# yangt1013/SPEINet

Hardware: AMD Instinct MI355X
Metric: deblurred 720p frames/sec (higher is better)
Workload: dtype f16 (correlation top2)

## Files before the change

### include/speinet_hip.h

```cpp
#ifndef SPEINET_HIP_H
#define SPEINET_HIP_H

#include <stdint.h>

#ifdef __cplusplus
extern "C" {
#endif

typedef void* spei_stream_t;

#define SPEI_ACT_NONE 0
#define SPEI_ACT_RELU 1
#define SPEI_ACT_GELU 2

#define SPEI_F32 0
#define SPEI_BF16 1
#define SPEI_F16 2

#define SPEI_CONV 0
#define SPEI_CONV_TRANSPOSED 1

int spei_version(void);
const char* spei_last_error(void);
const char* spei_arch(void);

int spei_any_nonzero(const float* x, int64_t n, int32_t* flag, spei_stream_t stream);

int spei_rl_prior(const float* img, float* out, float* scratch, int C, int H, int W, int iters, float lam,
                  spei_stream_t stream);

int spei_conv5_in(const float* img_chw, const float* w, const float* bias, float* out_hwc, int H, int W,
                  int Cout, spei_stream_t stream);

int spei_conv5_out(const float* in_hwc, int ldi, const float* w, const float* bias, float* out_chw, int H,
                   int W, int Cin, spei_stream_t stream);

int spei_igemm_f32(const float* a0, int lda0, int k0, const float* a1, int lda1, int k1, const float* w,
                   const float* bias, float* out, int ldo, const float* residual, int ldr,
                   const float* rowscale, int Hin, int Win, int Hout, int Wout, int N, int ksize, int stride,
                   int pad, int mode, int act, spei_stream_t stream);

int spei_igemm_f32_batched(const float* a0, int lda0, int k0, const float* a1, int lda1, int k1, const float* w,
                           const float* bias, float* out, int ldo, const float* residual, int ldr,
                           const float* rowscale, int Hin, int Win, int Hout, int Wout, int N, int ksize, int stride,
                           int pad, int mode, int act, int batch, spei_stream_t stream);

int spei_conv_slab16(int fmt, const void* a0, int lda0, int k0, const void* a1, int lda1, int k1, int a_fmt,
                     const void* wfrag_hi, const void* wfrag_lo, const float* bias, void* out, int ldo, int out_fmt,
                     const float* residual, int ldr, const float* rowscale, int Hin, int Win, int Hout, int Wout,
                     int N, int ksize, int stride, int pad, int act, int ln_input, spei_stream_t stream);

int spei_conv_slab16_batched(int fmt, const void* a0, int k0, int a_fmt, const void* wfrag, const void* wfrag_lo, const float* bias,
                             void* out, int out_fmt, const float* residual, int batch, int Hin, int Win, int Hout, int Wout, int N,
                             int ksize, int stride, int pad, int act, spei_stream_t stream);

int spei_conv32_ws16(int fmt, const void* a, int a_fmt, const void* wfrag, const float* bias, void* out, int out_fmt, int batch,
                     int H, int W, int act, spei_stream_t stream);

int spei_conv64_ws16(int fmt, const void* a, int a_fmt, const void* wfrag, const float* bias, void* out, int out_fmt, int batch,
                     int H, int W, int act, spei_stream_t stream);

int spei_mlp_fused16(int fmt, const float* x, float* out, const void* w1_frag, const float* b1, const void* w2_frag,
                     const float* b2, int64_t M, spei_stream_t stream);

int spei_convt2_slab16(int fmt, const void* a0, int lda0, int k0, int a_fmt, const void* wfrag00, const void* wfrag01,
                       const void* wfrag10, const void* wfrag11, const float* bias, void* out, int ldo, int out_fmt,
                       int Hin, int Win, int N, int act, spei_stream_t stream);

int spei_convt2_slab16x3(const float* a0, int lda0, int k0, const void* const* whi4, const void* const* wlo4, const float* bias,
                         float* out, int ldo, int Hin, int Win, int N, int act, spei_stream_t stream);

int spei_conv3x3_256_pipe16(int fmt, const float* x, const void* w_frag, const float* bias, const float* residual, float* out,
                            int batch, int H, int W, spei_stream_t stream);

int spei_conv5_out_slab16(int fmt, const void* in, int ldi, int in_fmt, const void* wfrag, const float* bias32, float* out_chw,
                          int H, int W, spei_stream_t stream);

int spei_attn_fused16(int fmt, const float* x, float* out, const void* yhat, const void* wq_frag, const float* bq,
                      const void* wkv_frag, const float* bkv, const void* wproj_frag, const float* bproj,
                      const float* relbias, int H, int W, int shift, spei_stream_t stream);

int spei_attn_win4_16(int fmt, const float* x, float* out, const void* yhat, const void* wq_frag, const float* bq,
                      const void* wkv_frag, const float* bkv, const void* wproj_frag, const float* bproj,
                      const float* relbias, int batch, int H, int W, int shift, spei_stream_t stream);

int64_t spei_frame_metrics_ws_doubles(int H, int W, int border);
int spei_frame_metrics(const unsigned char* out_hwc, const unsigned char* gt_hwc, int H, int W, int border, double* ws, double* result,
                       spei_stream_t stream);

int64_t spei_gate_ws_floats(int H, int W, int C);
int spei_resblock_gates(const void* x1, int x1_fmt, int H, int W, int C, const float* se_w1, const float* se_b1,
                        const float* se_w2, const float* se_b2, const float* cw_w, const float* cw_bn,
                        const float* hc_w, const float* hc_bn, float* s, float* g1, float* g2, float* ws,
                        spei_stream_t stream);
int spei_resblock_apply(const float* x, const void* x1, int x1_fmt, const float* s, const float* g1, const float* g2,
                        const float* extra, float* out, int ldo, int H, int W, int C, spei_stream_t stream);

int spei_resblock_gates_batched(const void* x1, int x1_fmt, int batch, int H, int W, int C, const float* se_w1, const float* se_b1,
                                const float* se_w2, const float* se_b2, const float* cw_w, const float* cw_bn, const float* hc_w,
                                const float* hc_bn, float* s, float* g1, float* g2, float* ws, spei_stream_t stream);
int spei_resblock_apply_batched(const float* x, const void* x1, int x1_fmt, const float* s, const float* g1, const float* g2, float* out,
                                int batch, int H, int W, int C, spei_stream_t stream);

int spei_layernorm256(const float* x, void* y, int out_fmt, const float* gamma, const float* beta, int64_t M,
                      spei_stream_t stream);

int spei_window_attention(const void* q, const void* kv, int io_fmt, const float* relbias, void* out, int H, int W,
                          int shift, spei_stream_t stream);
int spei_window_attention_batched(const void* q, const void* kv, int io_fmt, const float* relbias, void* out, int H, int W,
                                  int shift, int batch, spei_stream_t stream);

int spei_patch_invnorm(const float* f, int ldf, float* inv, int H, int W, int C, spei_stream_t stream);

int64_t spei_corr_ws_floats(int64_t n_lr);
int spei_corr_argmax(const float* lr, int ldl, const float* ref, int ldr, const float* inv_lr,
                     const float* inv_ref, int Hl, int Wl, int Hr, int Wr, int C, float* S, int32_t* arg,
                     float* ws, spei_stream_t stream);

int spei_split16(int fmt, const float* x, int ld, void* hi, void* lo, int64_t M, int C, spei_stream_t stream);
int spei_corr_argmax_bf16(const void* lr_hi, const void* lr_lo, const void* ref_hi, const void* ref_lo,
                          const float* inv_lr, const float* inv_ref, int Hl, int Wl, int Hr, int Wr, int C, float* S,
                          int32_t* arg, float* ws, spei_stream_t stream);

int spei_corr_slab16(int fmt, const void* lr_hi, const void* lr_lo, const void* ref_hi, const void* ref_lo,
                     const float* inv_lr, const float* inv_ref, int Hl, int Wl, int Hr, int Wr, int C, float* S,
                     int32_t* arg, float* ws, spei_stream_t stream);

int spei_corr_slab_top2_16(int fmt, const void* lr16, const void* ref16, const float* inv_lr, const float* inv_ref,
                           int Hl, int Wl, int Hr, int Wr, int C, float* S, int32_t* arg, float* S2, int32_t* arg2,
                           float* ws, spei_stream_t stream);
int64_t spei_corr_diag_ws_floats(int Hl, int Wl, int Hr, int Wr);
int spei_corr_diag_top2_16(int fmt, const void* lr16, const void* ref16, const float* inv_ref, int Hl, int Wl, int Hr, int Wr,
                           int C, float* S, int32_t* arg, float* S2, int32_t* arg2, float* ws, spei_stream_t stream);
int spei_corr_rescore(const float* lr, int ldl, const float* ref, int ldr, const float* inv_lr, const float* inv_ref,
                      int Hl, int Wl, int Hr, int Wr, int C, float* S, int32_t* arg, const float* S2, const int32_t* arg2,
                      spei_stream_t stream);

int spei_gather_fold(const float* ref, int ldr, const int32_t* arg, float* out, int ldo, int H3, int W3,
                     int Hr3, int Wr3, int C, int s, spei_stream_t stream);

int spei_rot90(const float* in, int ldi, float* out, int H, int W, int C, spei_stream_t stream);

int spei_upsample_bicubic(const float* in, int ldi, float* out, int ldo, int H, int W, int C, int s, int act,
// ... 119 lines not shown
```

### speinet_amd/engine.py

```python
from __future__ import annotations

import torch

from .ops import ACT_GELU, ACT_RELU, CONV_T, BMap, Ctx, FMap


def _resblocks(ctx: Ctx, f: FMap, blocks, extra=None, out=None) -> FMap:
    n = len(blocks)
    for i, pk in enumerate(blocks):
        last = i == n - 1
        f = ctx.resblock(f, pk, extra=extra if last else None, out=out if last else None)
    return f


def in_block(ctx: Ctx, frame: torch.Tensor, pk: dict) -> FMap:
    ctx = ctx.for_stage("enc")
    return _resblocks(ctx, ctx.conv5_in(frame, pk["head_w"], pk["head_b"]), pk["blocks"])


def enc_stage(ctx: Ctx, f: FMap, pk: dict, extra=None, out=None) -> FMap:
    ctx = ctx.for_stage("enc")
    n = pk["head_b"].numel()
    f = ctx.igemm(f, pk["head_w"], pk["head_b"], n, ksize=5, stride=2, act=ACT_RELU)
    return _resblocks(ctx, f, pk["blocks"], extra, out)
# ... 86 lines not shown
        ctx.igemm(FMap(cur, h, w, 256), layer["conv_w"], layer["conv_b"], 256, ksize=3, residual=rf, out=rf)
    xt = ctx.layernorm(r, sw["norm_g"], sw["norm_b"])
    res = ctx.igemm(FMap(xt, h, w, 256), sw["cab_w"], sw["cab_b"], 256, ksize=3, residual=sx.x_first)
    return ctx.igemm(res, sw["conv_last_w"], sw["conv_last_b"], 128, ksize=3, residual=sx.f_mid, out=out)


def swin_multi(ctx: Ctx, sx: SwinX, feats: BMap, sw: dict, outs: list) -> None:
    ctx = ctx.for_stage("swin")
    B, h, w = feats.B, feats.H, feats.W
    m = h * w
    dev = feats.t.device
    y_first = ctx.igemm_batched(feats, sw["conv_first_w"], sw["conv_first_b"], 256, 3)
    yt = ctx.layernorm(y_first.t, sw["pe_g"], sw["pe_b"])
    idt = ctx.inter_dtype()
    yhat = ctx.layernorm(yt, out_dtype=idt)
    del y_first, yt
    r = sx.xt0.repeat(B, 1)
    bufs = [torch.empty(B * m, 256, device=dev), torch.empty(B * m, 256, device=dev)]
    for layer in sw["layers"]:
        cur = r
        for bi, bk in enumerate(layer["blocks"]):
            shift = 0 if bi % 2 == 0 else 2
            nxt = bufs[bi % 2]
            ctx.attn_fused(cur, yhat, bk, h, w, shift, out=nxt)
            ctx.mlp_fused(nxt, bk["w1"], bk["b1"], bk["w2"], bk["b2"], out=nxt)
            cur = nxt
        rb = BMap(r, B, h, w, 256)
        ctx.igemm_batched(BMap(cur, B, h, w, 256), layer["conv_w"], layer["conv_b"], 256, 3, residual=rb, out=rb)
    xt = ctx.layernorm(r, sw["norm_g"], sw["norm_b"])
    x_first = BMap(sx.x_first.t.repeat(B, 1), B, h, w, 256)
    res = ctx.igemm_batched(BMap(xt, B, h, w, 256), sw["cab_w"], sw["cab_b"], 256, 3, residual=x_first)
    for b in range(B):
        ctx.igemm(res.map(b), sw["conv_last_w"], sw["conv_last_b"], 128, ksize=3, residual=sx.f_mid, out=outs[b])


def search_plan(ctx: Ctx, f_fusion: FMap, lv3: FMap):
    ctx = ctx.for_stage("search")
    return ctx.corr_plan(f_fusion, lv3, ctx.patch_invnorm(f_fusion), ctx.patch_invnorm(lv3))


def search_finish(ctx: Ctx, plan, f_fusion: FMap, lv1: FMap, lv2: FMap, lv3: FMap, return_arg=False):
    ctx = ctx.for_stage("search")
    s, arg = plan.s, plan.arg
    if ctx.capture is not None:
        ctx.capture.update(arg=arg, s=s)
    h3, w3 = f_fusion.H, f_fusion.W
    t3 = ctx.gather_fold(lv3, arg, h3, w3, lv3.H, lv3.W, 1)
    t2 = ctx.gather_fold(lv2, arg, h3, w3, lv3.H, lv3.W, 2)
    t1 = ctx.gather_fold(lv1, arg, h3, w3, lv3.H, lv3.W, 4)
    if return_arg:
        return s, t3, t2, t1, arg
    return s, t3, t2, t1


def search_transfer(ctx: Ctx, f_fusion: FMap, lv1: FMap, lv2: FMap, lv3: FMap, return_arg=False):
    plan = search_plan(ctx, f_fusion, lv3)
    plan.launch()
    return search_finish(ctx, plan, f_fusion, lv1, lv2, lv3, return_arg)


def self_plan(ctx: Ctx, f_fusion: FMap):
    ctx = ctx.for_stage("search")
    ref = ctx.rot90(f_fusion)
    return ctx.corr_plan(f_fusion, ref, ctx.patch_invnorm(f_fusion), ctx.patch_invnorm(ref))


def self_finish(ctx: Ctx, plan, f_fusion: FMap, P: dict):
    ctx = ctx.for_stage("search")
    s = plan.s
    if ctx.capture is not None:
        ctx.capture.update(s_self=s)
    p1, p2 = P["SelfTransfer.search1"], P["SelfTransfer.search2"]
    t2 = ctx.up_conv1x1_relu(f_fusion, p1["w"], p1["b"], 64)
    t1 = ctx.up_conv1x1_relu(t2, p2["w"], p2["b"], 32)
    return s, f_fusion, t2, t1


def self_transfer(ctx: Ctx, f_fusion: FMap, P: dict):
    plan = self_plan(ctx, f_fusion)
    plan.launch()
    return self_finish(ctx, plan, f_fusion, P)


def decode(ctx: Ctx, ff: FMap, s: torch.Tensor, t3: FMap, t2: FMap, t1: FMap, P: dict, out: torch.Tensor) -> torch.Tensor:
    ctx = ctx.for_stage("decode")
    g = ctx.for_stage("glue")
    g1 = ctx.for_stage("glue1")
    c = lambda name: (P[name]["w"], P[name]["b"])
    h3, w3 = ff.H, ff.W
    smap = FMap(s.view(h3 * w3, 1), h3, w3, 1)
    f_lv3 = g.igemm(ff, *c("conv_lv3"), 128, a1=t3, rowscale=s, residual=ff)
    dec2 = dec_stage(ctx.for_stage("dec2"), f_lv3, P["decoder_second"])
    s2 = ctx.upsample(smap, 2).t.view(-1)
    f_lv2 = g.igemm(dec2, *c("conv_lv2"), 64, a1=t2, rowscale=s2, residual=dec2)
    s1 = g.up_conv1x1_relu(f_lv3, *c("search1"), 64)
    sr2 = g.igemm(f_lv2, *c("search3"), 64, ksize=3, act=ACT_RELU)
    f_v3 = g.igemm(dec2, *c("search2"), 64, a1=s1, act=ACT_RELU, residual=dec2)
    f_lv2 = g.igemm(f_lv2, *c("search2"), 64, a1=sr2, act=ACT_RELU, residual=f_lv2)
    dec1 = dec_stage(ctx.for_stage("dec1"), f_lv2, P["decoder_first"])
    s4 = ctx.upsample(smap, 4).t.view(-1)
    f_lv1 = g1.igemm(dec1, *c("conv_lv1"), 32, a1=t1, rowscale=s4, residual=dec1)
    s13 = g.up_conv1x1_relu(f_v3, *c("search13"), 32)
    s23 = g1.igemm(ctx.upsample(f_lv2, 2), *c("search33"), 32, ksize=3, act=ACT_RELU)
    s33 = g1.igemm(f_lv1, *c("search43"), 32, ksize=3, act=ACT_RELU)
    acc = g1.igemm(s13, *c("search33"), 32, ksize=3, a1=s23, act=ACT_RELU, residual=f_lv1)
    g1.igemm(s13, *c("search33"), 32, ksize=3, a1=s33, act=ACT_RELU, residual=acc, out=acc)
    g1.igemm(s23, *c("search33"), 32, ksize=3, a1=s33, act=ACT_RELU, residual=acc, out=acc)
    ob = P["outBlock"]
    ctx = ctx.for_stage("out")
    f = _resblocks(ctx, acc, ob["blocks"])
    return ctx.for_stage("tail").conv5_out(f, ob["tail_w"], ob["tail_b"], out, ob.get("tail_w32"), ob.get("tail_b32"))


def _lanes(ctx: Ctx, sides) -> list:
    return [torch.cuda.current_stream(ctx.device)] + list(sides or ())


def forward_sample(ctx: Ctx, x: torch.Tensor, P: dict, n_seq: int, has_ref: bool, out: torch.Tensor, sides=()) -> torch.Tensor:
    return _run(forward_sample_steps(ctx, x, P, n_seq, has_ref, out, sides), out)


def _run(steps, out):
    for plan in steps:
        plan.launch()
    return out


def forward_sample_steps(ctx: Ctx, x: torch.Tensor, P: dict, n_seq: int, has_ref: bool, out: torch.Tensor, sides=()):
    h, w = x.shape[-2:]
    h3, w3 = h // 4, w // 4
    dev = x.device
    lanes = _lanes(ctx, sides)
    main = lanes[0]
    if ctx.for_stage("enc").batched_available():
        yield from forward_batch_steps(ctx, x[None], P, n_seq, [not has_ref], out[None], sides)
        return
    for s_ in lanes[1:]:
        s_.wait_stream(main)
    lv = None
    if has_ref:
        with torch.cuda.stream(lanes[-1]):
            lv = reference_pyramid(ctx, x[n_seq + 1], P)
    cat = FMap(torch.empty(h3 * w3, 128 * n_seq, device=dev), h3, w3, 128 * n_seq)
    mid = x[n_seq // 2]
    e0 = enc(ctx, mid, P)
    f_mid = enc(ctx, ctx.rl_prior(mid, 5, 0.01), P, extra=e0, out=cat.view(0, 128))
    others = [i for i in range(n_seq) if i != n_seq // 2]
    if ctx.for_stage("swin").swin_multi_available():
        fb = BMap.empty(len(others), h3, w3, 128, dev)
        for k, i in enumerate(others):
            with torch.cuda.stream(lanes[k % len(lanes)]):
                e = enc(ctx, x[i], P)
                enc(ctx, ctx.rl_prior(x[i], 1, 0.01), P, extra=e, out=fb.map(k))
                del e
        for s_ in lanes[1:]:
            main.wait_stream(s_)
        yield from _fuse_tail(ctx, f_mid, fb, cat, lv, P, out, lanes)
        return
    sx = SwinX(ctx, f_mid, P["swin"])
    ready = torch.cuda.Event()
    ready.record(main)
    for slot, i in enumerate(others, start=1):
        lane = lanes[(slot - 1) % len(lanes)]
        with torch.cuda.stream(lane):
            e = enc(ctx, x[i], P)
            feat = enc(ctx, ctx.rl_prior(x[i], 1, 0.01), P, extra=e)
            if lane is not main:
                lane.wait_event(ready)
            swin(ctx, sx, feat, P["swin"], out=cat.view(128 * slot, 128))
            del e, feat
    for s_ in lanes[1:]:
        main.wait_stream(s_)
    yield from _tail(ctx, cat, lv, P, out)


def forward_batch_steps(ctx: Ctx, x: torch.Tensor, P: dict, n_seq: int, zero_ref: list, out: torch.Tensor, sides=(), max_maps: int = 16):
    B = x.shape[0]
    h, w = x.shape[-2:]
    h3, w3 = h // 4, w // 4
    dev = x.device
    lanes = _lanes(ctx, sides)
    main = lanes[0]
    others = [i for i in range(n_seq) if i != n_seq // 2]
    b0 = 0
    while b0 < B:
        group, maps = [], 0
        while b0 + len(group) < B:
            need = 2 + 2 * len(others) + (0 if zero_ref[b0 + len(group)] else 1)
            if group and maps + need > max_maps:
                break
# ... 122 lines not shown
```

### speinet_amd/ops.py

```python
from __future__ import annotations

import ctypes as C
import dataclasses
from typing import Optional

import numpy as np
import torch

from . import _lib
from .pack import BF16, F16, F32, LP_DTYPE, PackedW, fmt_of

ACT_NONE, ACT_RELU, ACT_GELU = 0, 1, 2
CONV, CONV_T = 0, 1

PRECISIONS = ("f32", "bf16x3", "bf16", "f16")
CORR_PRECISIONS = ("bf16x3", "single", "top2")
_CORR_ALIASES = {"bf16": "single", "bf16r": "top2", "f16": "single"}


class FMap:
    __slots__ = ("t", "H", "W", "C", "ld", "off")

    def __init__(self, t: torch.Tensor, H: int, W: int, C_: int, off: int = 0):
        assert t.is_cuda and t.dtype in (torch.float32, torch.bfloat16, torch.float16) and t.is_contiguous() and t.dim() == 2 and t.shape[0] == H * W
# ... 6 lines not shown

    @property
    def lp(self) -> bool:
        return self.t.dtype != torch.float32

    @property
    def fmt(self) -> int:
        return fmt_of(self.t.dtype)

    def view(self, off: int, C_: int) -> "FMap":
        return FMap(self.t, self.H, self.W, C_, self.off + off)

    @property
    def ptr(self) -> int:
        return self.t.data_ptr() + self.t.element_size() * self.off

    def dense(self) -> torch.Tensor:
        return self.t[:, self.off:self.off + self.C].float().reshape(self.H, self.W, self.C)

    def nchw(self) -> torch.Tensor:
        return self.dense().permute(2, 0, 1).unsqueeze(0).contiguous()

    @staticmethod
    def from_nchw(x: torch.Tensor) -> "FMap":
        if x.dim() == 4:
            x = x[0]
        c, h, w = x.shape
        return FMap(x.permute(1, 2, 0).reshape(h * w, c).contiguous().float(), h, w, c)


class BMap:
    __slots__ = ("t", "B", "H", "W", "C")

    def __init__(self, t: torch.Tensor, B: int, H: int, W: int, C_: int):
        assert t.is_cuda and t.is_contiguous() and t.shape == (B * H * W, C_)
        self.t, self.B, self.H, self.W, self.C = t, B, H, W, C_

    @staticmethod
    def empty(B: int, H: int, W: int, C_: int, device, dtype=torch.float32) -> "BMap":
        return BMap(torch.empty(B * H * W, C_, device=device, dtype=dtype), B, H, W, C_)

    @property
    def fmt(self) -> int:
        return fmt_of(self.t.dtype)

    def map(self, b: int) -> FMap:
        n = self.H * self.W
        return FMap(self.t[b * n:(b + 1) * n], self.H, self.W, self.C)


def _vp(p) -> C.c_void_p:
    return C.c_void_p(p)


class _timed:
    def __init__(self, ctx: "Ctx", name: str):
        self.on = ctx.profile is not None and name in ctx.profile
        self.ctx, self.name = ctx, name

    def __enter__(self):
        if self.on:
            self.s = torch.cuda.Event(enable_timing=True)
            self.e = torch.cuda.Event(enable_timing=True)
            self.s.record(torch.cuda.current_stream(self.ctx.device))
        return self

    def __exit__(self, *a):
        if self.on:
            self.e.record(torch.cuda.current_stream(self.ctx.device))
            self.ctx.profile[self.name].append((self.s, self.e))
        return False


def _tensor_bytes(x) -> int:
    t = x.t if hasattr(x, "t") else x
    return t.numel() * t.element_size() if torch.is_tensor(t) else 0


def _conv_sub(method: str, a, k, out):
    if method == "conv5_in":
        return "level1", 2.0 * 25 * 3 * 32 * a[0].shape[-2] * a[0].shape[-1], _tensor_bytes(a[0]) + _tensor_bytes(out)
    if method == "conv5_out":
        return "level1", 2.0 * 25 * 32 * 3 * a[0].H * a[0].W, _tensor_bytes(a[0]) + 12 * a[0].H * a[0].W
    src, n = a[0], a[3]
    ks = a[4] if len(a) > 4 else k.get("ksize", 1)
    if n == 32 and src.C == 32 and ks == 5 and k.get("stride", a[5] if len(a) > 5 else 1) == 1:
        maps = getattr(src, "B", 1)
        return "level1", 2.0 * 25 * 32 * 32 * maps * src.H * src.W, _tensor_bytes(src) + _tensor_bytes(out)
    return "rest", 0.0, 0


def _family(name: str):
    def deco(fn):
        def wrapper(self, *a, **k):
            pr = self.profile
            if pr is None or "families" not in pr:
                return fn(self, *a, **k)
            st = torch.cuda.current_stream(self.device)
            s_, e_ = torch.cuda.Event(enable_timing=True), torch.cuda.Event(enable_timing=True)
            s_.record(st)
            out = fn(self, *a, **k)
            e_.record(st)
            pr["families"].setdefault(name, []).append((s_, e_))
            if name == "conv":
                sub, fl, by = _conv_sub(fn.__name__, a, k, out)
                rec = pr.setdefault("conv_sub", {}).setdefault(sub, {"events": [], "flops": 0.0, "bytes": 0})
                rec["events"].append((s_, e_))
                rec["flops"] += fl
                rec["bytes"] += by
            return out
        wrapper.__name__, wrapper.__doc__ = fn.__name__, fn.__doc__
        return wrapper
    return deco


def frame_metrics(u8: torch.Tensor, gt_hwc: torch.Tensor, border: int = 4) -> torch.Tensor:
    assert u8.is_cuda and u8.dtype == torch.uint8 and u8.dim() == 3 and u8.shape[2] == 3 and u8.is_contiguous()
    h, w = u8.shape[:2]
    assert gt_hwc.shape == u8.shape and gt_hwc.dtype == torch.uint8 and gt_hwc.device == u8.device and gt_hwc.is_contiguous()
    lib = _lib.lib()
    n = lib.spei_frame_metrics_ws_doubles(h, w, border)
    if n < 0:
        raise ValueError(f"frame {w}x{h} with border {border} is smaller than the 11x11 SSIM window")
    dev = u8.device
    ws = torch.empty(n, dtype=torch.float64, device=dev)
    res = torch.empty(2, dtype=torch.float64, device=dev)
    with torch.cuda.device(dev):
        st = C.c_void_p(torch.cuda.current_stream(dev).cuda_stream)
        _lib.check(lib.spei_frame_metrics(_vp(u8.data_ptr()), _vp(gt_hwc.data_ptr()), h, w, border, _vp(ws.data_ptr()), _vp(res.data_ptr()),
                                          st), "spei_frame_metrics")
    return res


def padded_size(n: int) -> int:
    return -(-n // 20) * 20


def frames_u8_in(u8: torch.Tensor, out: Optional[torch.Tensor] = None, gray: bool = False, planes: bool = True):
    assert u8.is_cuda and u8.dtype == torch.uint8 and u8.dim() in (3, 4) and (planes or gray)
    fr = u8 if u8.dim() == 4 else u8.unsqueeze(0)
    n, h, w, c = fr.shape
    assert c == 3 and fr.stride()[1:] == (w * 3, 3, 1), "frames must be packed [H,W,3] (any frame stride)"
    hp, wp = padded_size(h), padded_size(w)
    dev = u8.device
    if planes:
        if out is None:
            out = torch.empty(n, 3, hp, wp, device=dev)
        assert out.is_cuda and out.device == dev and out.dtype == torch.float32 and out.is_contiguous() and out.numel() == n * 3 * hp * wp
    else:
        out = None
    g = torch.empty(n, h, w, device=dev) if gray else None
    lib = _lib.lib()
    with torch.cuda.device(dev):
        st = C.c_void_p(torch.cuda.current_stream(dev).cuda_stream)
        _lib.check(lib.spei_frames_u8_in(_vp(fr.data_ptr()), fr.stride(0), _vp(out.data_ptr() if out is not None else 0),
                                         _vp(g.data_ptr() if g is not None else 0), n, h, w, st), "spei_frames_u8_in")
    return out, g


def window_mean_u8(u8: torch.Tensor, starts, lengths, gray: bool = False, blur: Optional[torch.Tensor] = None,
                   gt: Optional[torch.Tensor] = None):
    assert u8.is_cuda and u8.dtype == torch.uint8 and u8.dim() == 4
    t, h, w, c = u8.shape
    assert c == 3 and u8.stride()[1:] == (w * 3, 3, 1), "frames must be packed [H,W,3] (any frame stride)"
    runs_host = torch.from_numpy(np.ascontiguousarray(np.stack([np.asarray(starts), np.asarray(lengths)], axis=1).astype(np.int32)))
    m = runs_host.shape[0]
# ... 23 lines not shown
    assert nonfinite is None or (nonfinite.device == x.device and nonfinite.dtype == torch.int32 and nonfinite.numel() >= 1)
    lib = _lib.lib()
    with torch.cuda.device(x.device):
        st = C.c_void_p(torch.cuda.current_stream(x.device).cuda_stream)
        _lib.check(lib.spei_frame_u8_out(_vp(x.data_ptr()), _vp(out.data_ptr()), _vp(nonfinite.data_ptr() if nonfinite is not None else 0),
                                         h, w, hp, wp, st), "spei_frame_u8_out")
    return out


def psnr_f32(a: torch.Tensor, b: torch.Tensor, shave: int = 4, rgb_range: float = 1.0) -> torch.Tensor:
    assert a.is_cuda and a.dtype == torch.float32 and a.dim() == 3 and a.shape[0] == 3 and a.is_contiguous()
    assert b.shape == a.shape and b.dtype == torch.float32 and b.device == a.device and b.is_contiguous()
    lib = _lib.lib()
    dev = a.device
    ws = torch.empty(PSNR_WS_DOUBLES, dtype=torch.float64, device=dev)
    res = torch.empty(2, dtype=torch.float64, device=dev)
    with torch.cuda.device(dev):
        st = C.c_void_p(torch.cuda.current_stream(dev).cuda_stream)
        _lib.check(lib.spei_psnr_f32(_vp(a.data_ptr()), _vp(b.data_ptr()), a.shape[1], a.shape[2], shave, float(rgb_range), _vp(ws.data_ptr()),
                                     _vp(res.data_ptr()), st), "spei_psnr_f32")
    return res


PSNR_WS_DOUBLES = 256


def psnr_of(sq_sum: float, count: float) -> float:
    import math
    mse = sq_sum / count
    return 100.0 if mse == 0 else 20 * math.log10(1.0 / math.sqrt(mse))


CORR_DIAG_WS_MAX = 8 << 30


class CorrPlan:
    __slots__ = ("ctx", "s", "arg", "kernel", "main", "post", "keep")

    def __init__(self, ctx, s, arg, kernel, main, post, keep):
        self.ctx, self.s, self.arg, self.kernel, self.main, self.post, self.keep = ctx, s, arg, kernel, main, post, keep

    def launch(self, profile: Optional[dict] = None) -> None:
        ctx = self.ctx if profile is None else self.ctx.replace(profile=profile)
        st = ctx._stream()
        if ctx.profile is not None:
            ctx.profile["corr_kernel"] = self.kernel
        fam = ctx.profile is not None and "families" in ctx.profile
        if fam:
            f0, f1 = torch.cuda.Event(enable_timing=True), torch.cuda.Event(enable_timing=True)
            f0.record(torch.cuda.current_stream(ctx.device))
        with _timed(ctx, "corr_argmax"):
            for fn, name, args in self.main:
                _lib.check(fn(*args, st), name)
        for fn, name, args in self.post:
            _lib.check(fn(*args, st), name)
        if fam:
            f1.record(torch.cuda.current_stream(ctx.device))
            ctx.profile["families"].setdefault("correlation", []).append((f0, f1))


@dataclasses.dataclass(frozen=True, slots=True, eq=False)
class Ctx:
    ACT_NONE, ACT_RELU, ACT_GELU = ACT_NONE, ACT_RELU, ACT_GELU
    CONV, CONV_T = CONV, CONV_T
    SPLIT_STAGES = ("glue", "dec2")

    precision: str = "f32"
    corr_precision: str = "bf16x3"
    device: Optional[torch.device] = None
    bf16_storage: bool = True
    x1_bf16: bool = True
    fuse_mlp: bool = True
    fuse_attn: bool = True
    commute_upconv: bool = True
    commute_any: bool = False
    corr_bf16: bool = True
    corr_diag: bool = True
    split_decode: bool = True
    batch_enc: bool = True
    attn_win4: bool = True
    conv32_ws: bool = True
    conv64_ws: Optional[bool] = None
    conv3_pipe: bool = True
    stage: Optional[dict] = None
    profile: Optional[dict] = None
    capture: Optional[dict] = None

    def __post_init__(self):
        put = object.__setattr__
        if self.precision not in PRECISIONS:
            raise ValueError(f"unknown precision {self.precision!r}")
        put(self, "corr_precision", _CORR_ALIASES.get(self.corr_precision, self.corr_precision))
        if self.corr_precision not in CORR_PRECISIONS:
            raise ValueError(f"unknown correlation precision {self.corr_precision!r}")
        cur = torch.cuda.current_device() if torch.cuda.is_available() else 0
        device = torch.device("cuda", cur) if self.device is None else torch.device(self.device)
        if device.type != "cuda":
            raise RuntimeError("speinet_amd runs on MI355X only (HIP kernels); there is no CPU path")
        put(self, "device", torch.device("cuda", cur) if device.index is None else device)
        for k in _BOOL_KNOBS:
            if type(getattr(self, k)) is not bool:
                put(self, k, bool(getattr(self, k)))
        if self.conv64_ws is not None:
            put(self, "conv64_ws", bool(self.conv64_ws))
        put(self, "stage", dict(self.stage) if self.stage else {})

    def replace(self, **kw) -> "Ctx":
        return dataclasses.replace(self, **kw)

    def for_stage(self, name: str) -> "Ctx":
        o = self.stage.get(name)
        if o is None and self.split_decode and self.precision == "f16" and name in self.SPLIT_STAGES:
            o = {"precision": "bf16x3", "commute_any": True}
        return self.replace(**o) if o else self

    def _tp(self, t: Optional[torch.Tensor]) -> C.c_void_p:
        if t is None:
            return C.c_void_p(0)
        assert t.is_cuda and t.is_contiguous()
        assert t.device == self.device, f"tensor on {t.device}, call context on {self.device}"
        return C.c_void_p(t.data_ptr())

    def _fp(self, f: Optional[FMap]) -> C.c_void_p:
        if f is None:
            return C.c_void_p(0)
        assert f.t.device == self.device, f"feature map on {f.t.device}, call context on {self.device}"
        return C.c_void_p(f.ptr)

    def _stream(self) -> C.c_void_p:
        assert torch.cuda.current_device() == self.device.index, \
            f"current device cuda:{torch.cuda.current_device()} != call context {self.device}"
        return C.c_void_p(torch.cuda.current_stream(self.device).cuda_stream)

    @property
    def lp16(self) -> bool:
        return self.precision in ("bf16", "f16")

    @property
    def fmt(self) -> int:
        return F16 if self.precision == "f16" else BF16

    def inter_dtype(self) -> torch.dtype:
        return LP_DTYPE[self.fmt] if (self.lp16 and self.bf16_storage) else torch.float32

    def any_nonzero(self, x: torch.Tensor, flag: torch.Tensor) -> None:
        _lib.check(_lib.lib().spei_any_nonzero(self._tp(x), x.numel(), self._tp(flag), self._stream()), "spei_any_nonzero")

    def train_batch(self, table: torch.Tensor, table_host: torch.Tensor, n_in: int, n_gt: int, input: torch.Tensor, gt: torch.Tensor,
                    patch: int, rgb_range: float = 1.0) -> None:
        nb = (n_in + n_gt) * 32
        assert table.dtype == torch.uint8 and table.numel() >= nb and not table_host.is_cuda and table_host.dtype == torch.uint8 \
            and table_host.is_contiguous() and table_host.numel() >= nb
        assert input.dtype == torch.float32 and input.numel() == n_in * 3 * patch * patch
        assert gt.dtype == torch.float32 and gt.numel() == n_gt * 3 * patch * patch
        _lib.check(_lib.lib().spei_train_batch_u8(self._tp(table), C.c_void_p(table_host.data_ptr()), n_in, n_gt, self._tp(input), self._tp(gt),
                                                  patch, float(rgb_range), self._stream()), "spei_train_batch_u8")

    def rl_prior(self, img: torch.Tensor, iters: int, lam: float = 0.01) -> torch.Tensor:
        c, h, w = img.shape
        out = torch.empty_like(img)
        scratch = torch.empty_like(img)
        _lib.check(_lib.lib().spei_rl_prior(self._tp(img), self._tp(out), self._tp(scratch), c, h, w, iters, lam, self._stream()),
                   "spei_rl_prior")
        return out

    @_family("conv")
# ... 29 lines not shown
                                     and out.t.data_ptr() != a.t.data_ptr()))
                and (residual is None or (residual.t.dtype == torch.float32 and getattr(residual, "ld", 256) == 256 and getattr(residual, "off", 0) == 0)))

    def _persistent_conv(self, a, w, bias, N: int, ksize: int, stride: int, act: int, residual, out, batch: int) -> bool:
        tp, lib, f = self._tp, _lib.lib(), self.fmt
        if self._conv3_pipe_ok(a, w, N, ksize, stride, act, residual, out):
            _lib.check(lib.spei_conv3x3_256_pipe16(f, tp(a.t), tp(w.frag(f)), tp(bias), tp(residual.t) if residual is not None else _vp(0),
                                                   tp(out.t), batch, a.H, a.W, self._stream()), "spei_conv3x3_256_pipe16")
            return True
        if not (ksize == 5 and stride == 1 and a.C == N and residual is None and act in (ACT_NONE, ACT_RELU) and w.fhi is not None
                and (getattr(a, "ld", N), getattr(a, "off", 0), getattr(out, "ld", N), getattr(out, "off", 0)) == (N, 0, N, 0)
                and a.t.data_ptr() != out.t.data_ptr()):
            return False
        if N == 32 and self.conv32_ws_available():
            _lib.check(lib.spei_conv32_ws16(f, tp(a.t), a.fmt, tp(w.frag(f)), tp(bias), tp(out.t), out.fmt, batch, a.H, a.W, act,
                                            self._stream()), "spei_conv32_ws16")
            return True
        if N == 64 and self.conv64_ws_available():
            _lib.check(lib.spei_conv64_ws16(f, tp(a.t), a.fmt, tp(w.frag(f)), tp(bias), tp(out.t), out.fmt, batch, a.H, a.W, act,
                                            self._stream()), "spei_conv64_ws16")
            return True
        return False

    @_family("conv")
    def igemm(self, a0: FMap, w, bias: Optional[torch.Tensor], N: int, ksize: int = 1, stride: int = 1,
              mode: int = CONV, act: int = ACT_NONE, a1: Optional[FMap] = None, residual: Optional[FMap] = None,
              rowscale: Optional[torch.Tensor] = None, out: Optional[FMap] = None, out_dtype=torch.float32,
              ln_input: bool = False) -> FMap:
        prec = self.precision
        pad = ksize // 2
        if mode == CONV:
            ho, wo = (a0.H + 2 * pad - ksize) // stride + 1, (a0.W + 2 * pad - ksize) // stride + 1
        else:
            ho, wo = a0.H * stride, a0.W * stride
        if out is None:
            out = FMap.empty(ho, wo, N, a0.t.device, out_dtype)
        assert out.H == ho and out.W == wo and out.C == N
        k0, k1 = a0.C, (a1.C if a1 is not None else 0)
        slab = prec != "f32" and mode == CONV
        assert slab or (mode == CONV_T and self.lp16) or not (a0.lp or out.lp), \
            "16-bit activations are only supported by the slab kernel"
        assert a1 is None or a1.t.dtype == a0.t.dtype
        assert residual is None or not residual.lp
        assert all(f.t.dtype in (torch.float32, LP_DTYPE[self.fmt]) for f in (a0, out)), "16-bit tensors must be in the mode's format"
        if torch.is_tensor(w):
            w = PackedW(w, a0.t.device)
        assert not ln_input or (slab and w.fhi is not None), "ln_input is a feature of the slab kernel"
        assert tuple(w.shape) == (ksize * ksize, N, k0 + k1), (tuple(w.shape), ksize, N, k0, k1)
        if a1 is not None:
            assert (a1.H, a1.W) == (a0.H, a0.W)
        if residual is not None:
            assert (residual.H, residual.W, residual.C) == (ho, wo, N)
        if rowscale is not None:
            assert rowscale.numel() == ho * wo
        tp, fp = self._tp, self._fp
        srcs = (fp(a0), a0.ld, k0, fp(a1), a1.ld if a1 is not None else 0, k1)
        lib = _lib.lib()
        if (mode == CONV and a1 is None and rowscale is None and not ln_input
                and self._persistent_conv(a0, w, bias, N, ksize, stride, act, residual, out, 1)):
            return out
        if (mode == CONV_T and self.lp16 and ksize == 3 and stride == 2 and a1 is None and residual is None
                and rowscale is None and N % 32 == 0 and k0 % 32 == 0):
            cf = w.convT_class_frags(self.fmt)
            _lib.check(lib.spei_convt2_slab16(self.fmt, fp(a0), a0.ld, k0, a0.fmt, tp(cf[(0, 0)]), tp(cf[(0, 1)]), tp(cf[(1, 0)]),
                                              tp(cf[(1, 1)]), tp(bias), fp(out), out.ld, out.fmt, a0.H, a0.W, N, act,
                                              self._stream()), "spei_convt2_slab16")
        elif (mode == CONV_T and prec == "bf16x3" and ksize == 3 and stride == 2 and a1 is None and residual is None
                and rowscale is None and N % 32 == 0 and k0 % 32 == 0 and not a0.lp and not out.lp):
            _hi, _lo, ph, pl = w.convT_class_frags_split()
            _lib.check(lib.spei_convt2_slab16x3(fp(a0), a0.ld, k0, ph, pl, tp(bias), fp(out), out.ld, a0.H, a0.W, N, act, self._stream()),
                       "spei_convt2_slab16x3")
        elif prec == "f32":
            _lib.check(lib.spei_igemm_f32(*srcs, tp(w.f32), tp(bias), fp(out), out.ld, fp(residual), residual.ld if residual is not None else 0,
                                          tp(rowscale), a0.H, a0.W, ho, wo, N, ksize, stride, pad, mode, act, self._stream()), "spei_igemm_f32")
        elif slab and w.fhi is not None:
            dims = (a0.H * a0.W, 1, ho * wo, 1) if (ksize == 1 and stride == 1) else (a0.H, a0.W, ho, wo)
            _lib.check(lib.spei_conv_slab16(
                self.fmt, *srcs, a0.fmt, tp(w.frag(self.fmt)), tp(w.flo) if prec == "bf16x3" else _vp(0), tp(bias), fp(out), out.ld,
                out.fmt, fp(residual), residual.ld if residual is not None else 0,
                tp(rowscale), *dims, N, ksize, stride, pad, act, int(ln_input), self._stream()), "spei_conv_slab16")
        else:
            raise ValueError(f"no {prec} kernel for N={N} K={k0 + k1} ksize={ksize} stride={stride} mode={mode}: N and K must be multiples "
                             "of 32; transposed convs 3x3 stride 2")
        return out

    def linear(self, x: torch.Tensor, w, b: Optional[torch.Tensor], act: int = ACT_NONE,
               residual: Optional[torch.Tensor] = None, out: Optional[torch.Tensor] = None, out_dtype=torch.float32,
               ln_input: bool = False) -> torch.Tensor:
        m, k = x.shape
        if torch.is_tensor(w):
            w = PackedW(w.reshape(1, *w.shape), x.device)
        n = w.shape[1]
        if out is None:
            out = torch.empty(m, n, device=x.device, dtype=out_dtype)
        self.igemm(FMap(x, m, 1, k), w, b, n, act=act, ln_input=ln_input,
                   residual=FMap(residual, m, 1, n) if residual is not None else None, out=FMap(out, m, 1, n))
        return out

    @_family("streaming")
    def resblock_gates(self, x1: FMap, pk: dict):
        dev = x1.t.device
        lib = _lib.lib()
        tp = self._tp
        assert x1.off == 0 and x1.ld == x1.C
        s = torch.empty(x1.C, device=dev)
        g1 = torch.empty(x1.H, x1.C, device=dev)
        g2 = torch.empty(x1.W, x1.C, device=dev)
        ws = torch.empty(lib.spei_gate_ws_floats(x1.H, x1.W, x1.C), device=dev)
        _lib.check(lib.spei_resblock_gates(self._fp(x1), x1.fmt, x1.H, x1.W, x1.C, tp(pk["se_w1"]), tp(pk["se_b1"]), tp(pk["se_w2"]),
                                           tp(pk["se_b2"]), tp(pk["cw_w"]), tp(pk["cw_bn"]), tp(pk["hc_w"]), tp(pk["hc_bn"]),
                                           tp(s), tp(g1), tp(g2), tp(ws), self._stream()), "spei_resblock_gates")
        return s, g1, g2

    def resblock(self, x: FMap, pk: dict, extra: Optional[FMap] = None, out: Optional[FMap] = None) -> FMap:
        idt = self.inter_dtype()
        c = x.C
        assert x.off == 0 and x.ld == c
        t = self.igemm(x, pk["w1"], pk["b1"], c, ksize=5, act=ACT_RELU, out_dtype=idt)
        x1 = self.igemm(t, pk["w2"], pk["b2"], c, ksize=5, out_dtype=idt if self.x1_bf16 else torch.float32)
        s, g1, g2 = self.resblock_gates(x1, pk)
        if out is None:
            out = FMap.empty(x.H, x.W, c, x.t.device)
        if extra is not None:
            assert extra.off == 0 and extra.ld == c
        self._apply(x, x1, s, g1, g2, extra, out, c)
        return out

    @_family("streaming")
    def _apply(self, x, x1, s, g1, g2, extra, out, c):
        _lib.check(_lib.lib().spei_resblock_apply(self._fp(x), self._fp(x1), x1.fmt, self._tp(s), self._tp(g1), self._tp(g2),
                                                  self._fp(extra), self._fp(out), out.ld, x.H, x.W, c, self._stream()),
                   "spei_resblock_apply")

    def batched_available(self) -> bool:
        return self.batched_kernels() and self.x1_bf16 and self.bf16_storage and self.batch_enc

    def conv32_ws_available(self) -> bool:
        return self.lp16 and self.conv32_ws

    def conv64_ws_available(self) -> bool:
        return self.lp16 and (self.conv32_ws if self.conv64_ws is None else self.conv64_ws)

    def batched_kernels(self) -> bool:
        return self.lp16

    @_family("conv")
    def igemm_batched(self, a: BMap, w, bias: torch.Tensor, N: int, ksize: int, stride: int = 1, act: int = ACT_NONE,
                      out_dtype=torch.float32, residual: Optional[BMap] = None, out: Optional[BMap] = None) -> BMap:
        assert self.batched_kernels() and not torch.is_tensor(w) and w.fhi is not None
        pad = ksize // 2
        ho, wo = (a.H + 2 * pad - ksize) // stride + 1, (a.W + 2 * pad - ksize) // stride + 1
        assert tuple(w.shape) == (ksize * ksize, N, a.C) and a.t.dtype in (torch.float32, LP_DTYPE[self.fmt])
        if out is None:
            out = BMap.empty(a.B, ho, wo, N, a.t.device, out_dtype)
        assert (out.B, out.H, out.W, out.C) == (a.B, ho, wo, N) and out.t.data_ptr() != a.t.data_ptr()
        if residual is not None:
            assert (residual.B, residual.H, residual.W, residual.C) == (a.B, ho, wo, N) and residual.t.dtype == torch.float32
            assert residual.t.data_ptr() != a.t.data_ptr()
        tp = self._tp
        if self._persistent_conv(a, w, bias, N, ksize, stride, act, residual, out, a.B):
            return out
        _lib.check(_lib.lib().spei_conv_slab16_batched(self.fmt, tp(a.t), a.C, a.fmt, tp(w.frag(self.fmt)), _vp(0), tp(bias), tp(out.t), out.fmt,
                                                       tp(residual.t) if residual is not None else _vp(0), a.B, a.H, a.W, ho, wo, N, ksize,
                                                       stride, pad, act, self._stream()),
                   "spei_conv_slab16_batched")
        return out
# ... 182 lines not shown
```

Measured before the change: 41.55.

## Fuse three search33 pairwise conv launches into one persistent summing kernel

Replaces three sequential 3x3 conv launches, each reading a pair of the three 32-channel maps and accumulating ReLU output into a residual, with one persistent kernel. The kernel stages all three input tiles in LDS once, keeps the weights in registers, runs the three pairwise MFMA passes, and adds the residual in registers. Loading of the next tile's slabs is double-buffered and overlapped with the current passes. This removes two launches and the repeated read-modify-write of the fp32 accumulator and re-reads of the inputs, at the cost of a large LDS footprint (one block per CU) and hand-scheduled code.

```diff
diff --git a/include/speinet_hip.h b/include/speinet_hip.h
--- a/include/speinet_hip.h
+++ b/include/speinet_hip.h
@@ -59,6 +59,9 @@
 
 int spei_conv64_ws16(int fmt, const void* a, int a_fmt, const void* wfrag, const float* bias, void* out, int out_fmt, int batch,
                      int H, int W, int act, spei_stream_t stream);
+
+int spei_search_sum3_16(int fmt, const float* s13, const float* s23, const float* s33, const float* f_lv1, const void* wfrag,
+                        const float* bias, float* out, int H, int W, spei_stream_t stream);
 
 int spei_mlp_fused16(int fmt, const float* x, float* out, const void* w1_frag, const float* b1, const void* w2_frag,
                      const float* b2, int64_t M, spei_stream_t stream);
diff --git a/speinet_amd/csrc/search_sum16.hip b/speinet_amd/csrc/search_sum16.hip
--- /dev/null
+++ b/speinet_amd/csrc/search_sum16.hip
@@ -0,0 +1,224 @@
+#include "common.h"
+
+namespace {
+
+constexpr int C = 32, KS = 3, PAD = 1, NTAP = KS * KS, NSRC = 3;
+constexpr int TH = 8, TW = 32;
+constexpr int IH = TH + KS - 1, IW = TW + KS - 1;
+constexpr int PITCH = NSRC * 2 * C + 16;
+constexpr int SLAB = IH * IW * PITCH;
+constexpr int NTHR = 256, RT = 2;
+constexpr int KSTEPS = 2 * C / 16;
+constexpr int CPP = 8;
+constexpr int NCH = IH * IW * CPP;
+constexpr int NIT = (NCH + NTHR - 1) / NTHR;
+constexpr int PPI = NTHR / CPP;
+
+struct SumParams {
+    const float* src[NSRC];
+    const float* res;
+    const void* wfrag;
+    const float* bias;
+    float* out;
+    int H, W;
+    int tiles_x, total;
+};
+
+__device__ __forceinline__ void mfma_aw(f32x16& acc, const lpv<_Float16>::x8& w, const lpv<_Float16>::x8& b) {
+    asm volatile("v_mfma_f32_32x32x16_f16 %0, %1, %2, %0" : "+v"(acc) : "a"(w), "v"(b));
+}
+__device__ __forceinline__ void mfma_aw(f32x16& acc, const lpv<__bf16>::x8& w, const lpv<__bf16>::x8& b) {
+    asm volatile("v_mfma_f32_32x32x16_bf16 %0, %1, %2, %0" : "+v"(acc) : "a"(w), "v"(b));
+}
+
+template <typename LP>
+__global__ __launch_bounds__(NTHR, 1) void search_sum3_kernel(const SumParams p) {
+    typedef typename lpv<LP>::x8 lp8;
+    typedef typename lpv<LP>::x4 lp4;
+    extern __shared__ __attribute__((aligned(16))) unsigned char smem[];
+
+    const int tid = threadIdx.x, lane = tid & 63, wave = tid >> 6;
+    const int fr = lane & 31, fk = lane >> 5;
+
+    lp8 wreg[NTAP][KSTEPS];
+    {
+        const LP* wp = static_cast<const LP*>(p.wfrag) + lane * 8;
+#pragma unroll
+        for (int t = 0; t < NTAP; ++t)
+#pragma unroll
+            for (int s = 0; s < KSTEPS; ++s) wreg[t][s] = *reinterpret_cast<const lp8*>(wp + (t * KSTEPS + s) * 512);
+    }
+    float biasv[16];
+#pragma unroll
+    for (int r = 0; r < 16; ++r) biasv[r] = p.bias[8 * (r >> 2) + 4 * fk + (r & 3)];
+
+    typedef u32x4 stage_t;
+    stage_t sreg[NIT];
+
+    auto tile_origin = [&](int t, int& oy0, int& ox0) {
+        const int ty = t / p.tiles_x;
+        oy0 = ty * TH;
+        ox0 = (t - ty * p.tiles_x) * TW;
+    };
+    const int p0 = tid / CPP, sub = tid - p0 * CPP;
+    const int iy0 = p0 / IW, ix0 = p0 - iy0 * IW;
+    const int lds0 = p0 * PITCH + sub * 8;
+    auto advance = [](int& iy, int& ix) {
+        ix += PPI;
+        if (ix >= IW) { ix -= IW; ++iy; }
+    };
+    auto load_slab = [&](int t, int s) {
+        int oy0, ox0;
+        tile_origin(t, oy0, ox0);
+        const float* base = p.src[s] + sub * 4;
+        int iy = iy0, ix = ix0;
+#pragma unroll
+        for (int it = 0; it < NIT; ++it) {
+            const int iyc = min(iy, IH - 1);
+            const int gy = min(max(oy0 - PAD + iyc, 0), p.H - 1), gx = min(max(ox0 - PAD + ix, 0), p.W - 1);
+            sreg[it] = *reinterpret_cast<const stage_t*>(base + ((size_t)gy * p.W + gx) * C);
+            advance(iy, ix);
+        }
+    };
+    auto store_slab = [&](int t, int buf, int s) {
+        int oy0, ox0;
+        tile_origin(t, oy0, ox0);
+        unsigned char* sl = smem + buf * SLAB + lds0 + s * (2 * C);
+        int iy = iy0, ix = ix0;
+#pragma unroll
+        for (int it = 0; it < NIT; ++it) {
+            if (iy < IH) {
+                const bool ok = ((unsigned)(oy0 - PAD + iy) < (unsigned)p.H) & ((unsigned)(ox0 - PAD + ix) < (unsigned)p.W);
+                const f32x4 v = __builtin_bit_cast(f32x4, sreg[it]);
+                lp4 h = to_lp4<LP>(v);
+                if (!ok) h = lp4{(LP)0.f, (LP)0.f, (LP)0.f, (LP)0.f};
+                *reinterpret_cast<lp4*>(sl + it * PPI * PITCH) = h;
+            }
+            advance(iy, ix);
+        }
+    };
+
+    int t = blockIdx.x;
+    if (t >= p.total) return;
+#pragma unroll
+    for (int s = 0; s < NSRC; ++s) {
+        load_slab(t, s);
+        store_slab(t, 0, s);
+    }
+    lds_barrier();
+
+    int boff[RT];
+#pragma unroll
+    for (int i = 0; i < RT; ++i) boff[i] = ((wave * RT + i) * IW + fr) * PITCH + fk * 16;
+
+    int buf = 0;
+    for (; t < p.total; t += gridDim.x, buf ^= 1) {
+        const int tn = t + gridDim.x;
+        const int tl = tn < p.total ? tn : t;
+        int oy0, ox0;
+        tile_origin(t, oy0, ox0);
+        const int ox = ox0 + fr;
+        const int oxc = min(ox, p.W - 1);
+
+        f32x4 sum[RT][4];
+#pragma unroll
+        for (int i = 0; i < RT; ++i) {
+            const int oyc = min(oy0 + wave * RT + i, p.H - 1);
+            const float* r = p.res + ((size_t)oyc * p.W + oxc) * C + 4 * fk;
+#pragma unroll
+            for (int g = 0; g < 4; ++g) sum[i][g] = *reinterpret_cast<const f32x4*>(r + 8 * g);
+        }
+        load_slab(tl, 0);
+        __builtin_amdgcn_sched_barrier(0);
+
+        const unsigned char* sl = smem + buf * SLAB;
+        auto pass = [&](int a0, int a1) {
+            f32x16 acc[RT];
+#pragma unroll
+            for (int i = 0; i < RT; ++i)
+#pragma unroll
+                for (int r = 0; r < 16; ++r) acc[i][r] = biasv[r];
+            auto step_off = [&](int step) {
+                const int tap = step / KSTEPS, ks = step % KSTEPS;
+                return ((tap / KS) * IW + (tap % KS)) * PITCH + (ks < 2 ? a0 : a1) * (2 * C) + (ks & 1) * 32;
+            };
+            lp8 bq[3][RT];
+#pragma unroll
+            for (int d = 0; d < 2; ++d)
+#pragma unroll
+                for (int i = 0; i < RT; ++i) bq[d][i] = *reinterpret_cast<const lp8*>(sl + boff[i] + step_off(d));
+#pragma unroll
+            for (int step = 0; step < NTAP * KSTEPS; ++step) {
+                if (step + 2 < NTAP * KSTEPS) {
+#pragma unroll
+                    for (int i = 0; i < RT; ++i) bq[(step + 2) % 3][i] = *reinterpret_cast<const lp8*>(sl + boff[i] + step_off(step + 2));
+                }
+#pragma unroll
+                for (int i = 0; i < RT; ++i) mfma_aw(acc[i], wreg[step / KSTEPS][step % KSTEPS], bq[step % 3][i]);
+            }
+            __builtin_amdgcn_sched_barrier(0);
+            asm volatile("s_nop 7\n\ts_nop 7\n\ts_nop 7" ::: "memory");
+            __builtin_amdgcn_sched_barrier(0);
+#pragma unroll
+            for (int i = 0; i < RT; ++i)
+#pragma unroll
+                for (int r = 0; r < 16; ++r) sum[i][r >> 2][r & 3] = fmaxf(acc[i][r], 0.f) + sum[i][r >> 2][r & 3];
+        };
+
+        pass(0, 1);
+        store_slab(tl, buf ^ 1, 0);
+        load_slab(tl, 1);
+        __builtin_amdgcn_sched_barrier(0);
+        pass(0, 2);
+        store_slab(tl, buf ^ 1, 1);
+        load_slab(tl, 2);
+        __builtin_amdgcn_sched_barrier(0);
+        pass(1, 2);
+
+        if (ox < p.W) {
+#pragma unroll
+            for (int i = 0; i < RT; ++i) {
+                const int oy = oy0 + wave * RT + i;
+                if (oy < p.H) {
+                    float* o = p.out + ((size_t)oy * p.W + ox) * C + 4 * fk;
+#pragma unroll
+                    for (int g = 0; g < 4; ++g) *reinterpret_cast<f32x4*>(o + 8 * g) = sum[i][g];
+                }
+            }
+        }
+        store_slab(tl, buf ^ 1, 2);
+        lds_barrier();
+    }
+}
+
+template <typename LP>
+void launch_sum(const SumParams& p, hipStream_t st) {
+    const size_t lds = 2 * (size_t)SLAB;
+    const int cus = spei_num_cus();
+    const dim3 grid(p.total < cus ? p.total : cus);
+    ensure_dyn_lds<&search_sum3_kernel<LP>>(lds);
+    hipLaunchKernelGGL((search_sum3_kernel<LP>), grid, dim3(NTHR), lds, st, p);
+}
+
+}
+
+extern "C" int spei_search_sum3_16(int fmt, const float* s13, const float* s23, const float* s33, const float* f_lv1, const void* wfrag,
+                                   const float* bias, float* out, int H, int W, spei_stream_t stream) {
+    SPEI_REQUIRE(s13 && s23 && s33 && f_lv1 && wfrag && bias && out, "spei_search_sum3_16: null pointer");
+    SPEI_REQUIRE(fmt == SPEI_BF16 || fmt == SPEI_F16, "spei_search_sum3_16: fmt=%d", fmt);
+    SPEI_REQUIRE(H > 0 && W > 0 && (int64_t)H * W < (1ll << 26), "spei_search_sum3_16: map %dx%d", H, W);
+    SPEI_REQUIRE(((uintptr_t)s13 | (uintptr_t)s23 | (uintptr_t)s33 | (uintptr_t)f_lv1 | (uintptr_t)wfrag | (uintptr_t)out) % 16 == 0,
+                 "spei_search_sum3_16: 16-byte alignment");
+    const size_t bytes = (size_t)H * W * C * sizeof(float);
+    for (const float* in : {s13, s23, s33, f_lv1})
+        SPEI_REQUIRE((uintptr_t)out + bytes <= (uintptr_t)in || (uintptr_t)in + bytes <= (uintptr_t)out,
+                     "spei_search_sum3_16: out must not overlap an input");
+    SumParams p;
+    p.src[0] = s13; p.src[1] = s23; p.src[2] = s33; p.res = f_lv1; p.wfrag = wfrag; p.bias = bias; p.out = out; p.H = H; p.W = W;
+    p.tiles_x = cdiv(W, TW); p.total = p.tiles_x * cdiv(H, TH);
+    hipStream_t st = (hipStream_t)stream;
+    if (fmt == SPEI_F16) launch_sum<_Float16>(p, st);
+    else launch_sum<__bf16>(p, st);
+    SPEI_CHECK_LAUNCH("spei_search_sum3_16");
+    return 0;
+}
diff --git a/speinet_amd/engine.py b/speinet_amd/engine.py
--- a/speinet_amd/engine.py
+++ b/speinet_amd/engine.py
@@ -192,6 +192,15 @@
     return self_finish(ctx, plan, f_fusion, P)
 
 
+def search_sum(g1: Ctx, s13: FMap, s23: FMap, s33: FMap, f_lv1: FMap, w, b: torch.Tensor) -> FMap:
+    if g1.search_sum_available(s13, s23, s33, f_lv1):
+        return g1.search_sum(s13, s23, s33, f_lv1, w, b)
+    acc = g1.igemm(s13, w, b, 32, ksize=3, a1=s23, act=ACT_RELU, residual=f_lv1)
+    g1.igemm(s13, w, b, 32, ksize=3, a1=s33, act=ACT_RELU, residual=acc, out=acc)
+    g1.igemm(s23, w, b, 32, ksize=3, a1=s33, act=ACT_RELU, residual=acc, out=acc)
+    return acc
+
+
 def decode(ctx: Ctx, ff: FMap, s: torch.Tensor, t3: FMap, t2: FMap, t1: FMap, P: dict, out: torch.Tensor) -> torch.Tensor:
     ctx = ctx.for_stage("decode")
     g = ctx.for_stage("glue")
@@ -213,9 +222,7 @@
     s13 = g.up_conv1x1_relu(f_v3, *c("search13"), 32)
     s23 = g1.igemm(ctx.upsample(f_lv2, 2), *c("search33"), 32, ksize=3, act=ACT_RELU)
     s33 = g1.igemm(f_lv1, *c("search43"), 32, ksize=3, act=ACT_RELU)
-    acc = g1.igemm(s13, *c("search33"), 32, ksize=3, a1=s23, act=ACT_RELU, residual=f_lv1)
-    g1.igemm(s13, *c("search33"), 32, ksize=3, a1=s33, act=ACT_RELU, residual=acc, out=acc)
-    g1.igemm(s23, *c("search33"), 32, ksize=3, a1=s33, act=ACT_RELU, residual=acc, out=acc)
+    acc = search_sum(g1, s13, s23, s33, f_lv1, *c("search33"))
     ob = P["outBlock"]
     ctx = ctx.for_stage("out")
     f = _resblocks(ctx, acc, ob["blocks"])
diff --git a/speinet_amd/ops.py b/speinet_amd/ops.py
--- a/speinet_amd/ops.py
+++ b/speinet_amd/ops.py
@@ -112,6 +112,8 @@
         return "level1", 2.0 * 25 * 3 * 32 * a[0].shape[-2] * a[0].shape[-1], _tensor_bytes(a[0]) + _tensor_bytes(out)
     if method == "conv5_out":
         return "level1", 2.0 * 25 * 32 * 3 * a[0].H * a[0].W, _tensor_bytes(a[0]) + 12 * a[0].H * a[0].W
+    if method == "search_sum":
+        return "level1", 3 * 2.0 * 9 * 64 * 32 * a[0].H * a[0].W, sum(_tensor_bytes(x) for x in a[:4]) + _tensor_bytes(out)
     src, n = a[0], a[3]
     ks = a[4] if len(a) > 4 else k.get("ksize", 1)
     if n == 32 and src.C == 32 and ks == 5 and k.get("stride", a[5] if len(a) > 5 else 1) == 1:
@@ -301,6 +303,7 @@
     conv32_ws: bool = True
     conv64_ws: Optional[bool] = None
     conv3_pipe: bool = True
+    search_sum3: bool = True
     stage: Optional[dict] = None
     profile: Optional[dict] = None
     capture: Optional[dict] = None
@@ -496,6 +499,29 @@
         else:
             raise ValueError(f"no {prec} kernel for N={N} K={k0 + k1} ksize={ksize} stride={stride} mode={mode}: N and K must be multiples "
                              "of 32; transposed convs 3x3 stride 2")
+        return out
+
+    def search_sum_available(self, *maps: FMap) -> bool:
+        m0 = maps[0]
+        return (self.lp16 and self.search_sum3
+                and all((m.H, m.W, m.C, m.ld, m.off) == (m0.H, m0.W, 32, 32, 0) and m.t.dtype == torch.float32 for m in maps))
+
+    @_family("conv")
+    def search_sum(self, s13: FMap, s23: FMap, s33: FMap, f_lv1: FMap, w, bias: torch.Tensor, out: Optional[FMap] = None) -> FMap:
+        maps = (s13, s23, s33, f_lv1)
+        assert self.search_sum_available(*maps), "search_sum: single-product 16-bit mode, dense fp32 maps of 32 channels"
+        if torch.is_tensor(w):
+            w = PackedW(w, s13.t.device)
+        assert tuple(w.shape) == (9, 32, 64) and bias.numel() == 32
+        if out is None:
+            out = FMap.empty(s13.H, s13.W, 32, s13.t.device)
+        assert self.search_sum_available(s13, out)
+        store = out.t.untyped_storage().data_ptr()
+        if any(m.t.untyped_storage().data_ptr() == store for m in maps):
+            raise ValueError("search_sum: out must not alias an input (other tiles read every input's halo after a tile is written)")
+        fp = self._fp
+        _lib.check(_lib.lib().spei_search_sum3_16(self.fmt, fp(s13), fp(s23), fp(s33), fp(f_lv1), self._tp(w.frag(self.fmt)), self._tp(bias),
+                                                  fp(out), s13.H, s13.W, self._stream()), "spei_search_sum3_16")
         return out
 
     def linear(self, x: torch.Tensor, w, b: Optional[torch.Tensor], act: int = ACT_NONE,
```

After: 41.83 (median of 6 runs). About the same (+0.7%).
